# ming71/rotate-yolov3

Measured on AMD Instinct MI355X. Metric: images/sec fwd+bwd at 608^2 (train step, backend=hip), higher is better.
Workload: dtype bf16; 1 GPU; configs[3]: Darknet-53 train step (fwd + riou loss + bwd + grad all-reduce + SGD), bs=64/GPU 608x608, synthetic HRSC-shaped targets; global_batch=64, parallelism=dp1, gradients=250 MB fp32 in 4 flat buckets, fp32 on the wire

## Files before the change

rotate-yolov3_amd/csrc/conv.hip:

```cpp
#include <cstring>

#include <mutex>

#include "conv_common.h"

namespace ryolo_detail {
thread_local int *g_conv_choice = nullptr;
}

using namespace ryolo_detail;

namespace {

template <int KS, int BM, int BN, int WGM, int WGN, int NSTAGE, bool FAST, bool GEN, bool BNRED = false>
__global__ void __launch_bounds__(WGM *WGN * 64) conv_igemm_kernel(const ConvParams p, const BnRed br = BnRed()) {
    constexpr int NW = WGM * WGN, NT = NW * 64;
    constexpr int WPIX = BM / WGM, WCH = BN / WGN, PF = WPIX / 16, CF = WCH / 16;
    constexpr int A_BYTES = BM * BK * 2, B_BYTES = BN * BK * 2, STAGE = A_BYTES + B_BYTES;
    constexpr int A_PPW = (BM / 8) / NW, B_PPW = (BN / 8) / NW;
    static_assert(A_PPW >= 1 && B_PPW >= 1, "tile too small for the wave count");
    constexpr int SROW = BN * 2 + 16;
    static_assert(BM * SROW + WGM * 2 * BN * 4 <= NSTAGE * STAGE, "staging tile + statistics slots must fit in the operand buffers");
    constexpr int LOADS_PER_STAGE = A_PPW + B_PPW;

// ... 1992 lines not shown

int ryolo_conv_pack_job_fill(ryolo_pack_job *host_jobs , const float *w_oihw, int Cout, int Cin, int ksize,
                             int stride, int Cin_pad, void *packed_fwd, void *packed_dgrad ) {
    if (!host_jobs || !w_oihw || !packed_fwd || Cout <= 0 || Cin <= 0 || Cin_pad < Cin || (ksize != 1 && ksize != 3) ||
        (stride != 1 && stride != 2))
        return -1;
    int n = 0;
    {
        ryolo_pack_job &j = host_jobs[n++];
        j = ryolo_pack_job{};
        j.src = w_oihw; j.dst = packed_fwd; j.kind = 0; j.Cout = Cout; j.Cin = Cin; j.KS = ksize; j.Cin_pad = Cin_pad;
        j.Kpad = (ksize * ksize * Cin_pad + BK - 1) / BK * BK;
        j.rows = (Cout + 127) / 128 * 128;
        j.block_begin = 0; j.block_end = (j.rows + PK_ROWS - 1) / PK_ROWS;
        if (Cin * ksize * ksize > PK_LDS) return -1;
    }
    if (packed_dgrad) {
        if (ryolo_conv_packed_dgrad_bytes(Cout, Cin, ksize, stride) == 0) return -1;
        char *dst = (char *)packed_dgrad;
        for (int cls = 0; cls < (stride == 1 ? 1 : 4); cls++) {
            int dy[9], dx[9], khs[9], kws[9];
            const int nt = dgrad_classes(ksize, stride, (ksize - 1) / 2, cls, dy, dx, khs, kws);
            ryolo_pack_job &j = host_jobs[n++];
            j = ryolo_pack_job{};
            j.src = w_oihw; j.dst = dst; j.kind = 1; j.Cout = Cout; j.Cin = Cin; j.KS = ksize; j.ntaps = nt;
            for (int t = 0; t < nt; t++) { j.khs[t] = khs[t]; j.kws[t] = kws[t]; }
            j.Kpad = (nt * Cout + BK - 1) / BK * BK;
            j.rows = (Cin + 127) / 128 * 128;
            j.block_begin = 0; j.block_end = (j.rows / PK_CI) * ((Cout + PK_CO - 1) / PK_CO);
            dst += ((size_t)j.rows * j.Kpad + 128) * 2;
        }
        if (dgrad_xfusable(Cout, Cin, ksize, stride)) {
            for (int a = 0; a < 2; a++) {
                int dy[9], dx[9], khs[9], k0[9], k1[9];
                const int nt = dgrad_xfused_class(a, dy, dx, khs, k0, k1);
                ryolo_pack_job &j = host_jobs[n++];
                j = ryolo_pack_job{};
                j.src = w_oihw; j.dst = dst; j.kind = 2; j.Cout = Cout; j.Cin = Cin; j.KS = ksize; j.ntaps = nt;
                for (int t = 0; t < nt; t++) { j.khs[t] = khs[t]; j.kws[t] = (k0[t] + 1) | ((k1[t] + 1) << 4); }
                j.Kpad = (nt * Cout + BK - 1) / BK * BK;
                j.rows = (2 * Cin + 127) / 128 * 128;
                j.block_begin = 0; j.block_end = (j.rows / PK_CI) * ((Cout + PK_CO - 1) / PK_CO);
                dst += ((size_t)j.rows * j.Kpad + 128) * 2;
            }
        }
    }
    return n;
}

int ryolo_conv_pack_batch(const ryolo_pack_job *device_jobs, int njobs, int total_blocks, void *stream) {
    if (!device_jobs || njobs <= 0 || total_blocks <= 0) return RYOLO_EINVAL;
    hipLaunchKernelGGL(pack_batch_kernel, dim3((unsigned)total_blocks), dim3(256), 0, (hipStream_t)stream, device_jobs, njobs);
    return hipGetLastError() == hipSuccess ? RYOLO_OK : RYOLO_ELAUNCH;
}

int ryolo_conv_dgrad_tap_table(int ksize, int stride, int *host_out ) {
    if (!host_out || (ksize != 1 && ksize != 3) || (stride != 1 && stride != 2)) return RYOLO_EINVAL;
    for (int i = 0; i < 72; i++) host_out[i] = 0;
    for (int cls = 0; cls < (stride == 1 ? 1 : 4); cls++) {
        int dy[9], dx[9];
        dgrad_classes(ksize, stride, (ksize - 1) / 2, cls, dy, dx, host_out + cls * 18, host_out + cls * 18 + 9);
    }
    return RYOLO_OK;
}

int ryolo_conv_pack_weights_dgrad(const float *w_oihw, int Cout, int Cin, int ksize, int stride, void *packed,
                                  const int *taps_table , void *stream_) {
    if (!w_oihw || !packed || !taps_table || ryolo_conv_packed_dgrad_bytes(Cout, Cin, ksize, stride) == 0) return RYOLO_EINVAL;
    hipStream_t stream = (hipStream_t)stream_;
    const int rows = (Cin + 127) / 128 * 128;
    char *dst = (char *)packed;
    for (int cls = 0; cls < (stride == 1 ? 1 : 4); cls++) {
        int dy[9], dx[9], kk[18];
        const int nt = dgrad_classes(ksize, stride, (ksize - 1) / 2, cls, dy, dx, kk, kk + 9);
        const int Kpad = (nt * Cout + BK - 1) / BK * BK;
        const size_t total = (size_t)rows * Kpad + 128;
        const int nb = (int)((total + 255) / 256 < 4096 ? (total + 255) / 256 : 4096);
        hipLaunchKernelGGL(pack_dgrad_kernel, dim3(nb), dim3(256), 0, stream, w_oihw, Cout, Cin, ksize, nt,
                           taps_table + cls * 18, Kpad, rows, (__bf16 *)dst);
        dst += total * 2;
    }
    if (dgrad_xfusable(Cout, Cin, ksize, stride)) {
        const int rows2 = (2 * Cin + 127) / 128 * 128;
        for (int a = 0; a < 2; a++) {
            int dy[9], dx[9];
            XfTaps tp;
            const int nt = dgrad_xfused_class(a, dy, dx, tp.khs, tp.kw0, tp.kw1);
            for (int t = nt; t < 9; t++) { tp.khs[t] = 0; tp.kw0[t] = -1; tp.kw1[t] = -1; }
            const int Kpad = (nt * Cout + BK - 1) / BK * BK;
            const size_t total = (size_t)rows2 * Kpad + 128;
            const int nb = (int)((total + 255) / 256 < 4096 ? (total + 255) / 256 : 4096);
            hipLaunchKernelGGL(pack_dgrad_xfused_kernel, dim3(nb), dim3(256), 0, stream, w_oihw, Cout, Cin, nt, tp, Kpad, rows2,
                               (__bf16 *)dst);
            dst += total * 2;
        }
    }
    return hipGetLastError() == hipSuccess ? RYOLO_OK : RYOLO_ELAUNCH;
}

static int bnreduce_plan_tiles(const ryolo_conv_desc *d) {
    if (d->stride != 1 || (d->tile & 0xff) || d->in_cstride != d->Cin || (d->Cin & 7)) return 0;
    int knob = 1;
    {
        const char *e = tune(TUNE_BN_REDUCE_TILES);
        if (e) knob = atoi(e);
        if (knob == 0) return 0;
    }
    void *fake = (void *)(uintptr_t)4096;
    const BnRed *sv_b = g_bnred;
    const int sv_m = g_bnred_mode;
    int *sv_c = g_conv_choice;
    BnRed br{};
    int natural = -1, fused = -1;
    g_bnred = nullptr;
    g_conv_choice = &natural;
    int rc = ryolo_conv2d_dgrad(d, fake, d->Cout, fake, (const float *)fake, (const float *)fake, fake, 1, nullptr);
    if (rc == RYOLO_OK) {
        g_bnred = &br;
        g_bnred_mode = 3;
        g_conv_choice = &fused;
        rc = ryolo_conv2d_dgrad(d, fake, d->Cout, fake, (const float *)fake, (const float *)fake, fake, 1, nullptr);
    }
    g_bnred = sv_b;
    g_bnred_mode = sv_m;
    g_conv_choice = sv_c;
    if (rc != RYOLO_OK || natural != fused) return 0;
    const int tile = fused - RYOLO_CONV_KERNEL_IGEMM;
    const int bm = tile == 1 ? 128 : ((tile == 2 || tile == 3) ? 256 : 0);
    if (!bm) return 0;
    if (tile == 3) return 0;
    if (tile == 1 && knob == 2) return 0;
    const long long M = (long long)d->N * d->H * d->W;
    return (int)((M + bm - 1) / bm);
}

static int bnreduce_plan_mq128(const ryolo_conv_desc *d) {
    if (d->stride != 1 || (d->tile & 0xff) || d->in_cstride != d->Cin || (d->Cin & 127) || mq128_knob() <= 0) return 0;
    void *fake = (void *)(uintptr_t)4096;
    const BnRed *sv_b = g_bnred;
    int *sv_c = g_conv_choice;
    int natural = -1;
    g_bnred = nullptr;
    g_conv_choice = &natural;
    const int rc = ryolo_conv2d_dgrad(d, fake, d->Cout, fake, (const float *)fake, (const float *)fake, fake, 1, nullptr);
    g_bnred = sv_b;
    g_conv_choice = sv_c;
    if (rc != RYOLO_OK || (natural != RYOLO_CONV_KERNEL_MQ128 && natural != RYOLO_CONV_KERNEL_MQ64)) return 0;
    ConvParams q;
    q.M = (int)((long long)d->N * d->H * d->W);
    q.Cout = d->Cin;
    return conv_mq128_grid(q, natural == RYOLO_CONV_KERNEL_MQ128 ? 128 : 64);
}

static int bnreduce_plan(const ryolo_conv_desc *d, int *mode) {
    *mode = 0;
    if (validate(d) != RYOLO_OK) return 0;
    {
        const int r = bnreduce_plan_mq128(d);
        if (r > 0) {
            *mode = 4;
            return r;
        }
    }
    auto tiles = [&]() {
        const int r = bnreduce_plan_tiles(d);
        if (r > 0) *mode = 3;
        return r;
    };
    if (d->ksize != 1 || d->stride != 1 || d->pad != 0) return tiles();
    if ((d->Cin & 127) || (d->Cout & 63) || (d->tile & 0xff)) return tiles();
    const long long M = (long long)d->N * d->H * d->W;
    int g_pw = 0;
    {
        ConvParams q;
        q.Cin = d->Cout; q.Kpad = (d->Cout + BK - 1) / BK * BK; q.Cout = d->Cin; q.pw_grid_cap = 0;
        const int g = conv_pw_disabled() ? 0 : conv_pw_grid(q);
        if (g > 0 && d->in_cstride == d->Cin && ((unsigned long long)(M + 1024 * 128) * d->Cout) * 2ull < 0x7fffff00ull &&
            ((unsigned long long)M * d->Cin) * 2ull < 0x7fffff00ull)
            g_pw = g;
    }
    const long long mt = (M + 127) / 128, nt = d->Cin / 128, T = mt * nt;
    const int grid = (2 * cu_count()) & ~7;
    const long long dmax = d->W > d->H ? d->W : d->H;
    const bool persist_ok = !(grid < 8 || 2 * T < 5 * (long long)grid || mt * 128 * dmax >= 0x100000000ll || T * nt >= 0x100000000ll) &&
                            ((unsigned long long)M * d->Cout) * 2ull < 0x7fffff00ull;
    if (g_pw > 0 && (d->Cout == 128 || !persist_ok)) {
        *mode = 1;
        return g_pw;
    }
    if (persist_ok) {
        *mode = 2;
        return grid;
    }
    return tiles();
}

int ryolo_conv2d_dgrad_bnreduce_rows(const ryolo_conv_desc *d) {
    int mode;
    return bnreduce_plan(d, &mode);
}

int ryolo_conv2d_dgrad_bnreduce(const ryolo_conv_desc *d, const void *dz, int dz_cstride, const void *packed_dgrad, const float *ones,
                                const float *zeros, void *dx, int accumulate, const void *z, int z_cstride, const float *scale,
                                const float *shift, const float *mean, const float *invstd, const float *slope, float *part,
                                void *stream_) {
    int mode = 0;
    if (!bnreduce_plan(d, &mode) || !z || (z_cstride & 7) || z_cstride < d->Cin || !scale || !shift || !mean || !invstd ||
        !slope || !part || d->in_cstride != d->Cin)
        return RYOLO_EINVAL;
    BnRed br;
    br.z = (const __bf16 *)z; br.z_cs = z_cstride; br.scale = scale; br.shift = shift; br.mean = mean; br.invstd = invstd;
    br.slope = slope; br.part = part;
    g_bnred = &br;
    g_bnred_mode = mode;
    const int rc = ryolo_conv2d_dgrad(d, dz, dz_cstride, packed_dgrad, ones, zeros, dx, accumulate, stream_);
    g_bnred = nullptr;
    return rc;
}

int ryolo_conv2d_dgrad(const ryolo_conv_desc *d , const void *dz, int dz_cstride,
                       const void *packed_dgrad, const float *ones, const float *zeros, void *dx, int accumulate,
                       void *stream_) {
    if (validate(d) != RYOLO_OK || !dz || !packed_dgrad || !ones || !zeros || !dx) return RYOLO_EINVAL;
    if (d->stride != 1 && !(d->stride == 2 && d->ksize == 3 && d->pad == 1)) return RYOLO_EINVAL;
    if ((dz_cstride & 7) || dz_cstride < d->Cout) return RYOLO_EINVAL;
    const int Ho = (d->H + 2 * d->pad - d->ksize) / d->stride + 1, Wo = (d->W + 2 * d->pad - d->ksize) / d->stride + 1;
    const int rows = (d->Cin + 127) / 128 * 128;
    const char *wsrc = (const char *)packed_dgrad;
    const bool xfuse = dgrad_xfusable(d->Cout, d->Cin, d->ksize, d->stride) && d->pad == 1 && (d->W & 1) == 0 &&
                       d->in_cstride == d->Cin && !(d->tile & 0x8000);
    if (xfuse) wsrc += dgrad_classic_bytes(d->Cout, d->Cin, d->ksize, d->stride);
    if (!g_bnred && d->ksize == 3 && d->pad == 1 && ((d->Cin == 32 && d->Cout == 64) || (d->Cin == 64 && d->Cout == 128 && d->stride == 2)) &&
        !(d->tile & 0x80ff)) {
        const char *e = tune(TUNE_STEM_DGRAD);
        const int knob = e ? atoi(e) : 3;
        if (knob & (d->Cout == 64 ? 1 : 2)) {
            const int nt_out = (long long)d->N * d->H * d->W * d->Cin * 2 >= nt_out_min_bytes() ? 1 : 0;
            const unsigned long long dzb = (((unsigned long long)d->N * Ho * Wo - 1) * dz_cstride + d->Cout) * 2ull;
            const unsigned long long dxb = (((unsigned long long)d->N * d->H * d->W - 1) * d->in_cstride + d->Cin) * 2ull;
            if (dzb < 0x7fffff00ull && dxb < 0x7fffff00ull) {
                RYOLO_CONV_DRY_RUN(RYOLO_CONV_KERNEL_STEM_DGRAD);
                const int rc = launch_conv_stem_dgrad(d->Cout, d->stride, dz, dz_cstride, packed_dgrad, dx, d->in_cstride, accumulate, d->N, d->H,
                                                      d->W, nt_out, cu_count(), (hipStream_t)stream_);
                if (rc != RYOLO_EINVAL) return rc;
            }
        }
    }
    const int ncls = d->stride == 1 ? 1 : (xfuse ? 2 : 4);
    const int wrows = xfuse ? (2 * d->Cin + 127) / 128 * 128 : rows;
    for (int cls = 0; cls < ncls; cls++) {
        int dy[9], dxx[9], khs[9], kws[9];
        const int nt = xfuse ? dgrad_xfused_class(cls, dy, dxx, khs, kws, kws)
                             : dgrad_classes(d->ksize, d->stride, d->pad, cls, dy, dxx, khs, kws);
        ConvParams p;
        p.x = (const __bf16 *)dz;
        p.w = (const __bf16 *)wsrc;
        p.scale = ones; p.shift = zeros;
        p.res = accumulate ? (const __bf16 *)dx : nullptr;
        p.y = (__bf16 *)dx;
        p.N = d->N; p.H = Ho; p.W = Wo; p.Cin = d->Cout; p.in_cs = dz_cstride;
        p.Cout = d->Cin; p.out_cs = d->in_cstride; p.res_cs = d->in_cstride;
        p.K = nt * d->Cout;
        p.Kpad = (p.K + BK - 1) / BK * BK;
        p.act = RYOLO_ACT_LINEAR; p.slope = 0.f; p.ups = 1; p.nt = 0;
        p.cin_log2 = ilog2_exact(d->Cout);
        p.ntaps = nt;
        if (d->stride == 1) {
            p.stride = 1; p.pad = d->ksize - 1 - d->pad;
            p.Ho = d->H; p.Wo = d->W;
            for (int t = 0; t < nt; t++) { p.tap_dy[t] = dy[t]; p.tap_dx[t] = dxx[t]; }
            p.os = 1; p.osx = 1; p.ooy = 0; p.oox = 0; p.OH = d->H; p.OW = d->W;
        } else if (xfuse) {
            const int a = cls;
            p.stride = 1; p.pad = 0;
            p.Cout = 2 * d->Cin; p.out_cs = 2 * d->in_cstride; p.res_cs = 2 * d->in_cstride;
            p.Ho = (d->H - a + 1) / 2; p.Wo = d->W / 2;
            for (int t = 0; t < nt; t++) { p.tap_dy[t] = dy[t]; p.tap_dx[t] = dxx[t]; }
            p.os = 2; p.osx = 1; p.ooy = a; p.oox = 0; p.OH = d->H; p.OW = d->W / 2;
            if (p.Ho <= 0 || p.Wo <= 0) { wsrc += ((size_t)wrows * p.Kpad + 128) * 2; continue; }
        } else {
            const int a = cls >> 1, b = cls & 1;
            p.stride = 1; p.pad = 0;
            p.Ho = (d->H - a + 1) / 2; p.Wo = (d->W - b + 1) / 2;
            for (int t = 0; t < nt; t++) { p.tap_dy[t] = dy[t]; p.tap_dx[t] = dxx[t]; }
            p.os = 2; p.osx = 2; p.ooy = a; p.oox = b; p.OH = d->H; p.OW = d->W;
            if (p.Ho <= 0 || p.Wo <= 0) { wsrc += ((size_t)rows * p.Kpad + 128) * 2; continue; }
        }
        for (int t = nt; t < 9; t++) { p.tap_dy[t] = 0; p.tap_dx[t] = 0; }
        p.M = (int)((long long)d->N * p.Ho * p.Wo);
        const unsigned long long xb = (((unsigned long long)d->N * Ho * Wo - 1) * dz_cstride + d->Cout) * 2ull;
        const unsigned long long wb = ((unsigned long long)wrows * p.Kpad + 128) * 2ull;
        p.fast = (d->Cout % BK == 0) && xb < 0x7fffff00ull && wb < 0x7fffff00ull;
        p.taps2 = 0;
        if (!p.fast && (d->stride != 1 || (d->ksize == 3 && p.cin_log2 < 0))) return RYOLO_EINVAL;
        p.x_bytes = (unsigned)(p.fast ? xb : 0);
        p.w_bytes = (unsigned)(p.fast ? wb : 0);
        p.stat_part = nullptr; p.stat_cpad = 0;
        p.no_persist = (d->tile & 0x200) ? 1 : 0;
        p.force_persist = 0;
        p.pw_grid_cap = (d->tile & 0xff) == 13 ? (d->tile >> 16) & 0xff : 0;
        p.ntiles = 0; p.magic_wo = p.magic_ho = p.magic_nt = 0;
        p.nt_out = (long long)d->N * d->H * d->W * d->Cin * 2 >= nt_out_min_bytes() ? 1 : 0;
        const int pick = (d->tile & 0xff);
        const int rc = dispatch(p, d->ksize, pick, (hipStream_t)stream_);
        if (rc != RYOLO_OK) return rc;
        wsrc += ((size_t)wrows * p.Kpad + 128) * 2;
    }
    return RYOLO_OK;
}

}
```

rotate-yolov3_amd/csrc/conv_common.h:

```cpp
#pragma once
#include <hip/hip_runtime.h>
#include <stdint.h>
#include <stdlib.h>

#include "../../include/ryolo.h"

namespace ryolo_detail {

typedef __attribute__((ext_vector_type(8))) __bf16 bf16x8;
typedef __attribute__((ext_vector_type(4))) __bf16 bf16x4;
typedef __attribute__((ext_vector_type(2))) __bf16 bf16x2;
typedef __attribute__((ext_vector_type(4))) float f32x4;
typedef __attribute__((ext_vector_type(4))) unsigned int u32x4;
typedef __attribute__((address_space(3))) void *lds_vp;
typedef const __attribute__((address_space(1))) void *glb_vp;

constexpr int BK = 64;
constexpr long long NT_OUT_MIN_BYTES = 128ll << 20;
constexpr int STAT_ROWS = 128;

struct ConvParams {
    const __bf16 *x;
    const __bf16 *w;
    const float *scale;
    const float *shift;
    const __bf16 *res;
    __bf16 *y;
    int N, H, W, Cin, in_cs;
    int Ho, Wo, Cout, out_cs, res_cs;
    int stride, pad;
    int K, Kpad, M;
    int cin_log2;
    int act;
    float slope;
    int ups;
    int nt;
    unsigned x_bytes, w_bytes;
    int fast;
    int taps2;
    int no_persist;
    int force_persist;
    int ntaps;
    int tap_dy[9], tap_dx[9];
    int os, ooy, oox, OH, OW;
    int osx;
    int ntiles;
    unsigned magic_wo, magic_ho, magic_nt;
    int use_magic;
    unsigned y_bytes, res_bytes;
    double *stat_part;
    int stat_cpad;
    int nt_out;
    int reg3;
    int korder = 0;
    int dbg0, dbg1;
    int pw_nb, pw_mb;
    unsigned *trace;
    int pw_grid_cap;
};

struct BnRed {
    const __bf16 *z;
    int z_cs;
    const float *scale, *shift, *mean, *invstd;
    const float *slope;
    float *part;
    unsigned z_bytes = 0;
};

__device__ __forceinline__ float mish(float v) {
    const float e = __expf(fminf(v, 20.f));
    const float n = (1.f + e) * (1.f + e);
    return v * (n - 1.f) / (n + 1.f);
}

__device__ __forceinline__ float row16_sum(float v) {
#if defined(__HIP_DEVICE_COMPILE__)
    v += __builtin_bit_cast(float, __builtin_amdgcn_update_dpp(0, __builtin_bit_cast(int, v), 0xB1, 0xF, 0xF, true));
    v += __builtin_bit_cast(float, __builtin_amdgcn_update_dpp(0, __builtin_bit_cast(int, v), 0x4E, 0xF, 0xF, true));
    v += __builtin_bit_cast(float, __builtin_amdgcn_update_dpp(0, __builtin_bit_cast(int, v), 0x141, 0xF, 0xF, true));
    v += __builtin_bit_cast(float, __builtin_amdgcn_update_dpp(0, __builtin_bit_cast(int, v), 0x140, 0xF, 0xF, true));
#endif
    return v;
}

template <int O>
__device__ __forceinline__ float lane_xor_sum(float v) {
#if defined(__HIP_DEVICE_COMPILE__)
    if constexpr (O == 4) {
        v += __builtin_bit_cast(float, __builtin_amdgcn_update_dpp(0, __builtin_bit_cast(int, v), 0x124, 0xF, 0xF, true));
    } else if constexpr (O == 8) {
        v += __builtin_bit_cast(float, __builtin_amdgcn_update_dpp(0, __builtin_bit_cast(int, v), 0x128, 0xF, 0xF, true));
    } else if constexpr (O == 16) {
        const unsigned u = __builtin_bit_cast(unsigned, v);
        const auto s = __builtin_amdgcn_permlane16_swap(u, u, false, false);
        v = __builtin_bit_cast(float, (unsigned)s[0]) + __builtin_bit_cast(float, (unsigned)s[1]);
    } else {
        static_assert(O == 32, "partner distance");
        const unsigned u = __builtin_bit_cast(unsigned, v);
        const auto s = __builtin_amdgcn_permlane32_swap(u, u, false, false);
        v = __builtin_bit_cast(float, (unsigned)s[0]) + __builtin_bit_cast(float, (unsigned)s[1]);
    }
#endif
    return v;
}
template <int CPR>
__device__ __forceinline__ float lane_class_sum(float v) {
    if constexpr (CPR <= 4) v = lane_xor_sum<4>(v);
    if constexpr (CPR <= 8) v = lane_xor_sum<8>(v);
    v = lane_xor_sum<16>(v);
    return lane_xor_sum<32>(v);
}

__device__ __forceinline__ void buffer_load_lds16(const void *base, unsigned bytes, char *lds, int voffset, int soffset) {
#if defined(__HIP_DEVICE_COMPILE__)
    const __amdgpu_buffer_rsrc_t rsrc = __builtin_amdgcn_make_buffer_rsrc(const_cast<void *>(base), 0, bytes, 0x00020000);
    __builtin_amdgcn_raw_ptr_buffer_load_lds(rsrc, (lds_vp)lds, 16, voffset, soffset, 0, 0);
#endif
}

template <int AUX = 0>
__device__ __forceinline__ void buffer_store16_soff(u32x4 v, __amdgpu_buffer_rsrc_t rsrc, int voffset, int soffset) {
#if defined(__HIP_DEVICE_COMPILE__)
    __builtin_amdgcn_raw_buffer_store_b128(v, rsrc, voffset, soffset, AUX);
    asm volatile("s_nop 1" ::"v"(v));
#endif
}

__device__ __forceinline__ int udiv_magic(int n, unsigned magic) {
    return magic ? (int)__umulhi((unsigned)n, magic) : n;
}

__device__ __forceinline__ void split_pixel(int m, int Wo, int Ho, unsigned magic_wo, unsigned magic_ho, int use_magic, int &wo,
                                            int &ho, int &img) {
    if (use_magic) {
        const int t = udiv_magic(m, magic_wo);
        wo = m - t * Wo;
        img = udiv_magic(t, magic_ho);
        ho = t - img * Ho;
    } else {
        const int t = m / Wo;
        wo = m % Wo;
        ho = t % Ho;
        img = t / Ho;
    }
}


extern thread_local int *g_conv_choice;
#define RYOLO_CONV_DRY_RUN(code)          \
    do {                                  \
        if (ryolo_detail::g_conv_choice) { \
            *ryolo_detail::g_conv_choice = (code); \
            return RYOLO_OK;              \
        }                                 \
    } while (0)

int launch_conv_mp(ConvParams &p, int bm , int variant, hipStream_t stream);
int conv_mp_pick_bm(const ConvParams &p);
bool conv_mp_eligible(const ConvParams &p);
int launch_conv_mq(ConvParams &p, int variant, hipStream_t stream);
bool conv_mq128_eligible(const ConvParams &p);
int conv_mq128_grid(const ConvParams &p, int bm);
int launch_conv_mq128(ConvParams &p, int bm, const BnRed *bnred, hipStream_t stream);
bool conv_stem_eligible(const ConvParams &p, int ksize);
int launch_conv_stem(ConvParams &p, int cus, hipStream_t stream);
bool conv_stem64_eligible(const ConvParams &p, int ksize);
int launch_conv_stem64(ConvParams &p, int cus, hipStream_t stream);
int launch_conv0_halo(ConvParams &p, const float *slope_dev, int round_z, int cus, hipStream_t stream);
int launch_conv_stem_dgrad(int cdz, int stride, const void *dz, int dz_cs, const void *w_classes, void *dx, int dx_cs, int accumulate, int N,
                           int H, int W, int nt_out, int cus, hipStream_t stream);
int conv_stem_pair_kind(const ryolo_conv_desc *first, const ryolo_conv_desc *second, int shortcut_from_input);
int launch_conv_stem_pair(int kind, ConvParams &p , const void *x, unsigned x_bytes, int in_cs, int H, int W,
                          const void *w_first, int kpad_first, const float *scale_first, const float *shift_first, int act_first,
                          float slope_first, int cus, hipStream_t stream);
bool conv_pw_eligible(const ConvParams &p, int ksize);
bool conv_pw_preferred(const ConvParams &p);
int conv_pw_grid(const ConvParams &p);
int launch_conv_pw(ConvParams &p, const void *bnred , hipStream_t stream);
bool conv_pw_decode_supported(const ConvParams &p, int na, int no);
int launch_conv_pw_decode(ConvParams &p, float *io, long long io_img_rows, long long io_row0, float *pout, const float *anchors, int na, int no,
                          float stride, float cf, int arc, hipStream_t stream);
#ifdef RYOLO_MP_ABLATION
int ryolo_mp_ablation_variant(int slot);
#endif

enum TuneKey { TUNE_CONV3X3 = 0, TUNE_CONV1X1, TUNE_RNMS_TILES, TUNE_MQ_KORDER, TUNE_BN_REDUCE_TILES, TUNE_STEM_DGRAD, TUNE_COUNT };
const char *tune(TuneKey k);
#ifdef RYOLO_MP_ABLATION
inline const char *abl_env(const char *name) { return getenv(name); }
#else
inline const char *abl_env(const char *) { return nullptr; }
#endif

}
```

rotate-yolov3_amd/csrc/conv_stem.hip:

```cpp
#include <type_traits>

#include "conv_common.h"

namespace ryolo_detail {
namespace {

template <int N> using ic = std::integral_constant<int, N>;

constexpr int TW = 32;
constexpr int CIN = 32, COUT = 64, CG = COUT / 16;

template <int S>
struct Patch {
    static constexpr int TH = S == 1 ? 8 : 4;
    static constexpr int PH = (TH - 1) * S + 3, PW = (TW - 1) * S + 3, NPIX = PH * PW;
    static constexpr int NPIECE = (NPIX + 15) / 16;
    static constexpr int PPW = (NPIECE + 3) / 4;
    static constexpr int BUF = PPW * 4 * 1024;
    static constexpr int BYTES = 2 * BUF;
    static constexpr int GPW = TH * TW / 16 / 4;
};

__device__ __forceinline__ int chunk_swz(int pcol) { return (pcol ^ (pcol >> 2)) & 3; }

// ... 705 lines not shown
                }
            }
            f32x4 acc[2][2];
#pragma unroll
            for (int u = 0; u < 2; u++)
#pragma unroll
                for (int cg = 0; cg < 2; cg++) acc[u][cg] = f32x4{0.f, 0.f, 0.f, 0.f};
#pragma unroll
            for (int t = 0; t < 9; t++) {
                const int kh = t / 3, kw = t - 3 * kh;
#pragma unroll
                for (int ks = 0; ks < 2; ks++) {
                    bf16x8 xf[2];
#pragma unroll
                    for (int u = 0; u < 2; u++) {
                        const int pcol = u * 16 + fr + kw;
                        const int q = (jr + kh) * PW + pcol;
                        xf[u] = *(const bf16x8 *)(patch + q * 128 + (((ks * 4 + g) ^ swz(pcol)) << 4));
                    }
#pragma unroll
                    for (int u = 0; u < 2; u++)
#pragma unroll
                        for (int cg = 0; cg < 2; cg++)
                            acc[u][cg] = __builtin_amdgcn_mfma_f32_16x16x32_bf16(wfr[t][ks][cg], xf[u], acc[u][cg], 0, 0, 0);
                }
            }
#pragma unroll
            for (int u = 0; u < 2; u++) {
                unsigned o2[2][2];
#pragma unroll
                for (int cg = 0; cg < 2; cg++) {
                    bf16x4 o;
                    if constexpr (STATS) {
#pragma unroll
                        for (int rr = 0; rr < 4; rr++) {
                            o[rr] = (__bf16)acc[u][cg][rr];
                            const float qv = ok_[u] ? (float)o[rr] : 0.f;
                            st_sum[cg][rr] += qv;
                            st_sq[cg][rr] += qv * qv;
                        }
                    } else {
#pragma unroll
                        for (int rr = 0; rr < 4; rr++) {
                            float v = acc[u][cg][rr] * sc[cg][rr] + sh[cg][rr];
                            if constexpr (ACT == RYOLO_ACT_LEAKY) v = v > 0.f ? v : v * slope;
                            else if constexpr (ACT == RYOLO_ACT_MISH) v = mish(v);
                            o[rr] = (__bf16)v;
                        }
                    }
                    const uint2 uu = __builtin_bit_cast(uint2, o);
                    o2[cg][0] = uu.x;
                    o2[cg][1] = uu.y;
                }
#if defined(__HIP_DEVICE_COMPILE__)
#pragma unroll
                for (int d = 0; d < 2; d++) {
                    auto sw = __builtin_amdgcn_permlane16_swap(o2[0][d], o2[1][d], false, false);
                    o2[0][d] = sw[0];
                    o2[1][d] = sw[1];
                }
#endif
                u32x4 outv = u32x4{o2[0][0], o2[0][1], o2[1][0], o2[1][1]};
                if constexpr (!STATS) {
                    if (p.res) {
                        bf16x8 ov = __builtin_bit_cast(bf16x8, outv);
#pragma unroll
                        for (int e = 0; e < 8; e++) ov[e] = (__bf16)((float)ov[e] + (float)rv[u][e]);
                        outv = __builtin_bit_cast(u32x4, ov);
                    }
                }
                if (ok_[u]) {
                    u32x4 *dst = (u32x4 *)(p.y + (mbase + u * 16) * p.out_cs + co0 + run0);
                    if (p.nt_out) __builtin_nontemporal_store(outv, dst);
                    else *dst = outv;
                }
            }
        }
    }
    if constexpr (STATS) {
        float ta = 0.f, tb = 0.f;
#pragma unroll
        for (int cg = 0; cg < 2; cg++)
#pragma unroll
            for (int rr = 0; rr < 4; rr++) {
                const float a = row16_sum(st_sum[cg][rr]), b = row16_sum(st_sq[cg][rr]);
                if (fr == cg * 4 + rr) {
                    ta = a;
                    tb = b;
                }
            }
        if (fr < 8) {
            const int ch = co0 + (fr >> 2) * 16 + g * 4 + (fr & 3);
            double *row = p.stat_part + (size_t)(blockIdx.x % STAT_ROWS) * 2 * p.stat_cpad;
            atomicAdd(row + ch, (double)ta);
            atomicAdd(row + p.stat_cpad + ch, (double)tb);
        }
    }
}

template <bool STATS, int ACT>
int launch_stem64(ConvParams &p, int grid, int tiles_x, int tiles_y, int ntiles, hipStream_t stream) {
    hipLaunchKernelGGL((conv3x3_c64_halo_kernel<STATS, ACT>), dim3((unsigned)grid), dim3(256), c64::BYTES, stream, p, tiles_x, tiles_y, ntiles);
    return hipGetLastError() == hipSuccess ? RYOLO_OK : RYOLO_ELAUNCH;
}

template <int S, bool STATS>
int launch_stem(ConvParams &p, int grid, int tiles_x, int tiles_y, int ntiles, hipStream_t stream) {
    constexpr int smem = Patch<S>::BYTES;
    static bool attr_done = false;
    if (!attr_done) {
        if (smem > 64 * 1024 && hipFuncSetAttribute((const void *)conv3x3_c32_halo_kernel<S, STATS>,
                                                    hipFuncAttributeMaxDynamicSharedMemorySize, smem) != hipSuccess)
            return RYOLO_ELAUNCH;
        attr_done = true;
    }
    hipLaunchKernelGGL((conv3x3_c32_halo_kernel<S, STATS>), dim3((unsigned)grid), dim3(256), smem, stream, p, tiles_x, tiles_y, ntiles);
    return hipGetLastError() == hipSuccess ? RYOLO_OK : RYOLO_ELAUNCH;
}

}

bool conv_stem_eligible(const ConvParams &p, int ksize) {
    return ksize == 3 && p.Cin == CIN && p.Cout == COUT && p.pad == 1 && (p.stride == 1 || p.stride == 2) && p.fast && p.os == 1 &&
           p.ups == 1 && p.ntaps == 9 && (p.in_cs & 7) == 0 && (p.out_cs & 7) == 0 && (!p.res || (p.res_cs & 7) == 0) &&
           !(p.stat_part && p.res) && (long long)p.N * p.H * p.W * p.in_cs * 2 < 0x7fffff00ll;
}

bool conv_stem64_eligible(const ConvParams &p, int ksize) {
    return ksize == 3 && p.Cin == c64::CIN && p.Cout == c64::COUT && p.pad == 1 && p.stride == 1 && p.fast && p.os == 1 &&
           p.ups == 1 && p.ntaps == 9 && (p.in_cs & 7) == 0 && (p.out_cs & 7) == 0 && (!p.res || (p.res_cs & 7) == 0) &&
           !(p.stat_part && p.res) && (long long)p.N * p.H * p.W * p.in_cs * 2 < 0x7fffff00ll;
}

int launch_conv_stem64(ConvParams &p, int cus, hipStream_t stream) {
    const int tiles_x = (p.Wo + c64::TWX - 1) / c64::TWX, tiles_y = (p.Ho + c64::TH - 1) / c64::TH;
    const long long nt = (long long)p.N * tiles_x * tiles_y;
    if (nt > 0x7fffffffll) return RYOLO_EINVAL;
    RYOLO_CONV_DRY_RUN(RYOLO_CONV_KERNEL_STEM64);
    int grid = (2 * cus) & ~7;
    if (grid < 8) grid = 8;
    if (p.stat_part) return launch_stem64<true, RYOLO_ACT_LINEAR>(p, grid, tiles_x, tiles_y, (int)nt, stream);
    if (p.act == RYOLO_ACT_LEAKY) return launch_stem64<false, RYOLO_ACT_LEAKY>(p, grid, tiles_x, tiles_y, (int)nt, stream);
    if (p.act == RYOLO_ACT_MISH) return launch_stem64<false, RYOLO_ACT_MISH>(p, grid, tiles_x, tiles_y, (int)nt, stream);
    return launch_stem64<false, RYOLO_ACT_LINEAR>(p, grid, tiles_x, tiles_y, (int)nt, stream);
}

struct DgTile128 {
    static constexpr int TH = 8, TW = 32;
    static constexpr int PH = TH / 2 + 1, PW = TW / 2 + 1, NPIX = PH * PW;
    static constexpr int NPIECE = (NPIX + 3) / 4;
    static constexpr int PPW = (NPIECE + 3) / 4, BUF = PPW * 4 * 1024;
};

__global__ void __launch_bounds__(256, 2) dgrad3x3_s2_c128_kernel(const DgS2Params p) {
    using T = DgTile128;
    extern __shared__ __attribute__((aligned(16))) char smem[];
    const int tid = threadIdx.x, lane = tid & 63;
    const int wave = __builtin_amdgcn_readfirstlane(tid >> 6);
    const int fr = lane & 15, g = lane >> 4;
    const int q8 = p.ntiles >> 3, r8 = p.ntiles & 7, xcd = blockIdx.x & 7, loc = blockIdx.x >> 3, nloc = gridDim.x >> 3;
    const int start = xcd < r8 ? xcd * (q8 + 1) : r8 * (q8 + 1) + (xcd - r8) * q8;
    const int len = q8 + (xcd < r8 ? 1 : 0);
    bf16x8 wf[9][4];
    {
        constexpr int NCLS = 4;
        const __bf16 *img = p.w;
        int t0 = 0;
#pragma unroll
        for (int cls = 0; cls < NCLS; cls++) {
            const int nt = cls == 0 ? 1 : (cls == 3 ? 4 : 2), kpad = nt * 128;
#pragma unroll
            for (int t = 0; t < 4; t++) {
                if (t >= nt) break;
#pragma unroll
                for (int ks = 0; ks < 4; ks++) wf[t0 + t][ks] = *(const bf16x8 *)(img + (size_t)(wave * 16 + fr) * kpad + t * 128 + ks * 32 + g * 8);
            }
            t0 += nt;
            img += 128 * kpad + 128;
        }
    }
    const int tiles_img = p.tiles_x * p.tiles_y;
    auto fill = [&](int id, char *buf) {
        const int img = id / tiles_img, rem = id - img * tiles_img;
        const int ty = rem / p.tiles_x, tx = rem - ty * p.tiles_x;
        const int h0 = ty * (T::TH / 2), w0 = tx * (T::TW / 2);
#pragma unroll 2
        for (int j = 0; j < T::PPW; j++) {
            const int piece = wave * T::PPW + j;
            const int q = piece * 4 + (lane >> 4);
            const int prow = q / T::PW, pcol = q - prow * T::PW;
            const int ho = h0 + prow, wo = w0 + pcol;
            const bool ok = q < T::NPIX && (unsigned)ho < (unsigned)p.Ho && (unsigned)wo < (unsigned)p.Wo;
            const int chunk = (lane & 15) ^ (pcol & 15);
            const int off = (((img * p.Ho + ho) * p.Wo + wo) * p.dz_cs + chunk * 8) * 2;
            buffer_load_lds16(p.dz, p.dz_bytes, buf + piece * 1024, ok ? off : (int)0x80000000, 0);
        }
    };
    typedef __attribute__((ext_vector_type(2))) unsigned int u32x2;
    int cur = 0;
    if (loc < len) fill(start + loc, smem);
    for (int i = loc; i < len; i += nloc) {
        const int id = start + i;
        const int img = id / tiles_img, rem = id - img * tiles_img;
        const int ty = rem / p.tiles_x, tx = rem - ty * p.tiles_x;
        const int hi0 = ty * T::TH, wi0 = tx * T::TW;
        asm volatile("s_waitcnt vmcnt(0)" ::: "memory");
        __syncthreads();
        if (i + nloc < len) fill(id + nloc, smem + (cur ^ 1) * T::BUF);
        const char *patch = smem + cur * T::BUF;
        cur ^= 1;
        auto group = [&](auto Ac, auto Bc, auto T0c, int r) {
            constexpr int A = decltype(Ac)::value, B = decltype(Bc)::value, T0 = decltype(T0c)::value;
            constexpr int NTA = A ? 2 : 1, NTB = B ? 2 : 1;
            const int hi = hi0 + r, wi = wi0 + 2 * fr + B;
            const bool ok = hi < p.H && wi < p.W;
            const size_t m = ((size_t)img * p.H + hi) * p.W + wi;
            const int coff = wave * 16 + g * 4;
            u32x2 rv = u32x2{0u, 0u};
            if (p.res && ok) rv = *(const u32x2 *)(p.res + m * p.dx_cs + coff);
            f32x4 acc = f32x4{0.f, 0.f, 0.f, 0.f};
#pragma unroll
            for (int ta = 0; ta < NTA; ta++)
#pragma unroll
                for (int tb = 0; tb < NTB; tb++) {
                    const int prow = (r - A) / 2 + (A ? ta : 0), pcol = fr + (B ? tb : 0);
                    const char *px = patch + (prow * T::PW + pcol) * 256;
                    const int sw = pcol & 15;
#pragma unroll
                    for (int ks = 0; ks < 4; ks++) {
                        const bf16x8 xf = *(const bf16x8 *)(px + (((g + 4 * ks) ^ sw) << 4));
                        acc = __builtin_amdgcn_mfma_f32_16x16x32_bf16(wf[T0 + ta * NTB + tb][ks], xf, acc, 0, 0, 0);
                    }
                }
            bf16x4 o;
#pragma unroll
            for (int rr = 0; rr < 4; rr++) o[rr] = (__bf16)acc[rr];
            if (p.res) {
                const bf16x4 rb = __builtin_bit_cast(bf16x4, rv);
#pragma unroll
                for (int rr = 0; rr < 4; rr++) o[rr] = (__bf16)((float)o[rr] + (float)rb[rr]);
            }
            if (ok) {
                u32x2 *dst = (u32x2 *)(p.dx + m * p.dx_cs + coff);
                if (p.nt_out) __builtin_nontemporal_store(__builtin_bit_cast(u32x2, o), dst);
                else *dst = __builtin_bit_cast(u32x2, o);
            }
        };
        {
#pragma unroll
            for (int rp = 0; rp < T::TH / 2; rp++) {
                group(ic<0>{}, ic<0>{}, ic<0>{}, 2 * rp);
                group(ic<0>{}, ic<1>{}, ic<1>{}, 2 * rp);
                group(ic<1>{}, ic<0>{}, ic<3>{}, 2 * rp + 1);
                group(ic<1>{}, ic<1>{}, ic<5>{}, 2 * rp + 1);
            }
        }
    }
}

int launch_conv_stem_dgrad(int cdz, int stride, const void *dz, int dz_cs, const void *w_classes, void *dx, int dx_cs, int accumulate, int N,
                           int H, int W, int nt_out, int cus, hipStream_t stream) {
    const int Ho = stride == 2 ? (H - 1) / 2 + 1 : H, Wo = stride == 2 ? (W - 1) / 2 + 1 : W;
    const unsigned long long dzb = (((unsigned long long)N * Ho * Wo - 1) * dz_cs + cdz) * 2ull;
    if ((stride != 1 && stride != 2) || (cdz != 64 && !(cdz == 128 && stride == 2)) || dzb >= 0x7fffff00ull || (dz_cs & 7) || (dx_cs & 7) || dz_cs < cdz ||
        dx_cs < cdz / 2)
        return RYOLO_EINVAL;
    DgS2Params q;
    q.dz = (const __bf16 *)dz; q.dz_bytes = (unsigned)dzb; q.dz_cs = dz_cs; q.w = (const __bf16 *)w_classes;
    q.dx = (__bf16 *)dx; q.dx_cs = dx_cs; q.res = accumulate ? (const __bf16 *)dx : nullptr;
    q.H = H; q.W = W; q.Ho = Ho; q.Wo = Wo;
    const int th = cdz == 64 ? (stride == 2 ? DgTile<2>::TH : DgTile<1>::TH) : DgTile128::TH;
    const int tw = cdz == 64 ? (stride == 2 ? DgTile<2>::TW : DgTile<1>::TW) : DgTile128::TW;
    q.tiles_x = (W + tw - 1) / tw; q.tiles_y = (H + th - 1) / th;
    const long long nt = (long long)q.tiles_x * q.tiles_y * N;
    if (nt >= 0x7fffffff) return RYOLO_EINVAL;
    q.ntiles = (int)nt; q.nt_out = nt_out;
    int grid = (2 * cus) & ~7;
    if (grid < 8) grid = 8;
    if (cdz == 64) {
        if (stride == 2) hipLaunchKernelGGL(dgrad3x3_c64_kernel<2>, dim3((unsigned)grid), dim3(256), 2 * DgTile<2>::BUF, stream, q);
        else hipLaunchKernelGGL(dgrad3x3_c64_kernel<1>, dim3((unsigned)grid), dim3(256), 2 * DgTile<1>::BUF, stream, q);
    } else {
        hipLaunchKernelGGL(dgrad3x3_s2_c128_kernel, dim3((unsigned)grid), dim3(256), 2 * DgTile128::BUF, stream, q);
    }
    return hipGetLastError() == hipSuccess ? RYOLO_OK : RYOLO_ELAUNCH;
}

int launch_conv0_halo(ConvParams &p, const float *slope_dev, int round_z, int cus, hipStream_t stream) {
    if (!p.y || p.stat_part) return RYOLO_EINVAL;
    const int tiles_x = (p.Wo + C0_TW - 1) / C0_TW, tiles_y = (p.Ho + C0_TH - 1) / C0_TH;
    const long long nt = (long long)p.N * tiles_x * tiles_y;
    if (nt > 0x7fffffffll) return RYOLO_EINVAL;
    int grid = (4 * cus) & ~7;
    if (grid < 8) grid = 8;
    return launch_conv0_halo_t(p, slope_dev, round_z, p.act, grid, tiles_x, tiles_y, (int)nt, stream);
}

int launch_conv_stem(ConvParams &p, int cus, hipStream_t stream) {
    const int th = p.stride == 1 ? Patch<1>::TH : Patch<2>::TH;
    const int tiles_x = (p.Wo + TW - 1) / TW, tiles_y = (p.Ho + th - 1) / th;
    const long long nt = (long long)p.N * tiles_x * tiles_y;
    if (nt > 0x7fffffffll) return RYOLO_EINVAL;
    RYOLO_CONV_DRY_RUN(RYOLO_CONV_KERNEL_STEM);
    int grid = (2 * cus) & ~7;
    if (grid < 8) grid = 8;
    if (p.stat_part) return p.stride == 1 ? launch_stem<1, true>(p, grid, tiles_x, tiles_y, (int)nt, stream)
                                          : launch_stem<2, true>(p, grid, tiles_x, tiles_y, (int)nt, stream);
    return p.stride == 1 ? launch_stem<1, false>(p, grid, tiles_x, tiles_y, (int)nt, stream)
                         : launch_stem<2, false>(p, grid, tiles_x, tiles_y, (int)nt, stream);
}

static int launch_pair(ConvParams &p, const PairFirst &f, int cus, hipStream_t stream) {
    using G = PairGeom;
    const int tiles_x = (p.Wo + TW - 1) / TW, tiles_y = (p.Ho + G::P::TH - 1) / G::P::TH;
    const long long nt = (long long)p.N * tiles_x * tiles_y;
    if (nt > 0x7fffffffll) return RYOLO_EINVAL;
    static bool attr_done = false;
    if (!attr_done) {
        if (G::BYTES > 64 * 1024 && hipFuncSetAttribute((const void *)conv_stem_pair_kernel, hipFuncAttributeMaxDynamicSharedMemorySize,
                                                        G::BYTES) != hipSuccess)
            return RYOLO_ELAUNCH;
        attr_done = true;
    }
    int grid = (2 * cus) & ~7;
    if (grid < 8) grid = 8;
    hipLaunchKernelGGL(conv_stem_pair_kernel, dim3((unsigned)grid), dim3(256), G::BYTES, stream, p, f, tiles_x, tiles_y, (int)nt);
    return hipGetLastError() == hipSuccess ? RYOLO_OK : RYOLO_ELAUNCH;
}

int conv_stem_pair_kind(const ryolo_conv_desc *a, const ryolo_conv_desc *b, int shortcut_from_input) {
    if (!a || !b || a->upsample != 1 || b->upsample != 1 || a->N != b->N) return 0;
    const int aho = (a->H + 2 * a->pad - a->ksize) / a->stride + 1, awo = (a->W + 2 * a->pad - a->ksize) / a->stride + 1;
    if (aho != b->H || awo != b->W || a->Cout != b->Cin || b->Cin != CIN || b->Cout != COUT || b->ksize != 3 || b->pad != 1) return 0;
    if ((long long)a->N * a->H * a->W * a->in_cstride * 2 >= 0x7fffff00ll) return 0;
    if (a->ksize == 1 && a->stride == 1 && a->pad == 0 && a->Cin == 64 && b->stride == 1 && shortcut_from_input && (a->in_cstride & 7) == 0) return 2;
    return 0;
}

int launch_conv_stem_pair(int kind, ConvParams &p, const void *x, unsigned x_bytes, int in_cs, int H, int W, const void *w_first, int kpad_first,
                          const float *scale_first, const float *shift_first, int act_first, float slope_first, int cus, hipStream_t stream) {
    PairFirst f;
    f.x = (const __bf16 *)x; f.w = (const __bf16 *)w_first; f.scale = scale_first; f.shift = shift_first; f.x_bytes = x_bytes;
    f.in_cs = in_cs; f.Kpad = kpad_first; f.act = act_first; f.slope = slope_first; f.H = H; f.W = W;
    (void)kind;
    return launch_pair(p, f, cus, stream);
}

}
```

Before: 1381 images/s.

## Fuse BN/leaky-ReLU backward reduction into stride-2 stem dgrad kernel

Adds a BN-reduce mode to the specialized 3x3 stride-2 C128 stem dgrad kernel. The kernel now loads the pre-activation z, applies the leaky-ReLU gradient mask, and accumulates the per-channel BN backward partial sums in-kernel, writing per-block partials. Previously that layer either used the generic dgrad path with reduction or ran a separate reduction pass. The change avoids re-reading dx and z, at the cost of extra register pressure and z loads inside the stem kernel.

```diff
diff --git a/rotate-yolov3_amd/csrc/conv.hip b/rotate-yolov3_amd/csrc/conv.hip
--- a/rotate-yolov3_amd/csrc/conv.hip
+++ b/rotate-yolov3_amd/csrc/conv.hip
@@ -2168,9 +2168,32 @@
     return conv_mq128_grid(q, natural == RYOLO_CONV_KERNEL_MQ128 ? 128 : 64);
 }
 
+static int bnreduce_plan_stem(const ryolo_conv_desc *d) {
+    if (d->ksize != 3 || d->pad != 1 || d->stride != 2 || d->Cin != 64 || d->Cout != 128 || (d->tile & 0x80ff) || d->in_cstride != d->Cin) return 0;
+    {
+        const char *e = tune(TUNE_BN_REDUCE_TILES);
+        if (e && atoi(e) == 0) return 0;
+        const char *s = tune(TUNE_STEM_DGRAD);
+        if (!((s ? atoi(s) : 3) & 2)) return 0;
+    }
+    const int Ho = (d->H - 1) / 2 + 1, Wo = (d->W - 1) / 2 + 1;
+    const unsigned long long dzb = (((unsigned long long)d->N * Ho * Wo - 1) * d->Cout + d->Cout) * 2ull;
+    const unsigned long long dxb = (((unsigned long long)d->N * d->H * d->W - 1) * d->in_cstride + d->Cin) * 2ull;
+    if (dzb >= 0x7fffff00ull || dxb >= 0x7fffff00ull) return 0;
+    if ((long long)((d->W + 31) / 32) * ((d->H + 7) / 8) * d->N >= 0x7fffffff) return 0;
+    return conv_stem_dgrad_grid(cu_count());
+}
+
 static int bnreduce_plan(const ryolo_conv_desc *d, int *mode) {
     *mode = 0;
     if (validate(d) != RYOLO_OK) return 0;
+    {
+        const int r = bnreduce_plan_stem(d);
+        if (r > 0) {
+            *mode = 5;
+            return r;
+        }
+    }
     {
         const int r = bnreduce_plan_mq128(d);
         if (r > 0) {
@@ -2246,8 +2269,9 @@
     const bool xfuse = dgrad_xfusable(d->Cout, d->Cin, d->ksize, d->stride) && d->pad == 1 && (d->W & 1) == 0 &&
                        d->in_cstride == d->Cin && !(d->tile & 0x8000);
     if (xfuse) wsrc += dgrad_classic_bytes(d->Cout, d->Cin, d->ksize, d->stride);
-    if (!g_bnred && d->ksize == 3 && d->pad == 1 && ((d->Cin == 32 && d->Cout == 64) || (d->Cin == 64 && d->Cout == 128 && d->stride == 2)) &&
-        !(d->tile & 0x80ff)) {
+    const bool stem_red = g_bnred && g_bnred_mode == 5;
+    if ((!g_bnred || stem_red) && d->ksize == 3 && d->pad == 1 &&
+        ((d->Cin == 32 && d->Cout == 64 && !stem_red) || (d->Cin == 64 && d->Cout == 128 && d->stride == 2)) && !(d->tile & 0x80ff)) {
         const char *e = tune(TUNE_STEM_DGRAD);
         const int knob = e ? atoi(e) : 3;
         if (knob & (d->Cout == 64 ? 1 : 2)) {
@@ -2257,11 +2281,12 @@
             if (dzb < 0x7fffff00ull && dxb < 0x7fffff00ull) {
                 RYOLO_CONV_DRY_RUN(RYOLO_CONV_KERNEL_STEM_DGRAD);
                 const int rc = launch_conv_stem_dgrad(d->Cout, d->stride, dz, dz_cstride, packed_dgrad, dx, d->in_cstride, accumulate, d->N, d->H,
-                                                      d->W, nt_out, cu_count(), (hipStream_t)stream_);
-                if (rc != RYOLO_EINVAL) return rc;
-            }
-        }
-    }
+                                                      d->W, nt_out, cu_count(), stem_red ? g_bnred : nullptr, (hipStream_t)stream_);
+                if (rc != RYOLO_EINVAL || stem_red) return rc;
+            }
+        }
+    }
+    if (stem_red) return RYOLO_EINVAL;
     const int ncls = d->stride == 1 ? 1 : (xfuse ? 2 : 4);
     const int wrows = xfuse ? (2 * d->Cin + 127) / 128 * 128 : rows;
     for (int cls = 0; cls < ncls; cls++) {
diff --git a/rotate-yolov3_amd/csrc/conv_common.h b/rotate-yolov3_amd/csrc/conv_common.h
--- a/rotate-yolov3_amd/csrc/conv_common.h
+++ b/rotate-yolov3_amd/csrc/conv_common.h
@@ -169,7 +169,8 @@
 int launch_conv_stem64(ConvParams &p, int cus, hipStream_t stream);
 int launch_conv0_halo(ConvParams &p, const float *slope_dev, int round_z, int cus, hipStream_t stream);
 int launch_conv_stem_dgrad(int cdz, int stride, const void *dz, int dz_cs, const void *w_classes, void *dx, int dx_cs, int accumulate, int N,
-                           int H, int W, int nt_out, int cus, hipStream_t stream);
+                           int H, int W, int nt_out, int cus, const BnRed *bnred, hipStream_t stream);
+int conv_stem_dgrad_grid(int cus);
 int conv_stem_pair_kind(const ryolo_conv_desc *first, const ryolo_conv_desc *second, int shortcut_from_input);
 int launch_conv_stem_pair(int kind, ConvParams &p , const void *x, unsigned x_bytes, int in_cs, int H, int W,
                           const void *w_first, int kpad_first, const float *scale_first, const float *shift_first, int act_first,
diff --git a/rotate-yolov3_amd/csrc/conv_stem.hip b/rotate-yolov3_amd/csrc/conv_stem.hip
--- a/rotate-yolov3_amd/csrc/conv_stem.hip
+++ b/rotate-yolov3_amd/csrc/conv_stem.hip
@@ -881,7 +881,8 @@
     static constexpr int PPW = (NPIECE + 3) / 4, BUF = PPW * 4 * 1024;
 };
 
-__global__ void __launch_bounds__(256, 2) dgrad3x3_s2_c128_kernel(const DgS2Params p) {
+template <bool BNRED>
+__global__ void __launch_bounds__(256, 2) dgrad3x3_s2_c128_kernel(const DgS2Params p, const BnRed br) {
     using T = DgTile128;
     extern __shared__ __attribute__((aligned(16))) char smem[];
     const int tid = threadIdx.x, lane = tid & 63;
@@ -926,8 +927,31 @@
         }
     };
     typedef __attribute__((ext_vector_type(2))) unsigned int u32x2;
+    float bs1[4], bs2[4], bs3[4];
+    const float bn_slope = BNRED ? br.slope[0] : 0.f;
+    const float *bn_cst = (const float *)(smem + 2 * T::BUF);
+#pragma unroll
+    for (int rr = 0; rr < 4; rr++) bs1[rr] = bs2[rr] = bs3[rr] = 0.f;
+    if constexpr (BNRED) {
+        if (tid < 192) ((float *)(smem + 2 * T::BUF))[tid] = (tid < 64 ? br.scale : (tid < 128 ? br.shift : br.mean))[tid & 63];
+    }
+    u32x2 zq[4] = {u32x2{0u, 0u}, u32x2{0u, 0u}, u32x2{0u, 0u}, u32x2{0u, 0u}};
+    auto zreq = [&](int id2, int r, int B) -> u32x2 {
+        const int img2 = id2 / tiles_img, rem2 = id2 - img2 * tiles_img;
+        const int ty2 = rem2 / p.tiles_x, tx2 = rem2 - ty2 * p.tiles_x;
+        const int hi = ty2 * T::TH + r, wi = tx2 * T::TW + 2 * fr + B;
+        u32x2 v = u32x2{0u, 0u};
+        if (hi < p.H && wi < p.W) v = *(const u32x2 *)(br.z + (((size_t)img2 * p.H + hi) * p.W + wi) * br.z_cs + wave * 16 + g * 4);
+        return v;
+    };
     int cur = 0;
-    if (loc < len) fill(start + loc, smem);
+    if (loc < len) {
+        if constexpr (BNRED) {
+#pragma unroll
+            for (int k = 0; k < 4; k++) zq[k] = zreq(start + loc, k >> 1, k & 1);
+        }
+        fill(start + loc, smem);
+    }
     for (int i = loc; i < len; i += nloc) {
         const int id = start + i;
         const int img = id / tiles_img, rem = id - img * tiles_img;
@@ -938,9 +962,9 @@
         if (i + nloc < len) fill(id + nloc, smem + (cur ^ 1) * T::BUF);
         const char *patch = smem + cur * T::BUF;
         cur ^= 1;
-        auto group = [&](auto Ac, auto Bc, auto T0c, int r) {
-            constexpr int A = decltype(Ac)::value, B = decltype(Bc)::value, T0 = decltype(T0c)::value;
-            constexpr int NTA = A ? 2 : 1, NTB = B ? 2 : 1;
+        auto group = [&](auto Ac, auto Bc, auto T0c, auto RPc) {
+            constexpr int A = decltype(Ac)::value, B = decltype(Bc)::value, T0 = decltype(T0c)::value, RP = decltype(RPc)::value;
+            constexpr int NTA = A ? 2 : 1, NTB = B ? 2 : 1, r = 2 * RP + A;
             const int hi = hi0 + r, wi = wi0 + 2 * fr + B;
             const bool ok = hi < p.H && wi < p.W;
             const size_t m = ((size_t)img * p.H + hi) * p.W + wi;
@@ -974,21 +998,63 @@
                 if (p.nt_out) __builtin_nontemporal_store(__builtin_bit_cast(u32x2, o), dst);
                 else *dst = __builtin_bit_cast(u32x2, o);
             }
+            if constexpr (BNRED) {
+                const f32x4 bsc = *(const f32x4 *)(bn_cst + coff), bsh = *(const f32x4 *)(bn_cst + 64 + coff), bmu = *(const f32x4 *)(bn_cst + 128 + coff);
+                if (ok) {
+                    const bf16x4 zb = __builtin_bit_cast(bf16x4, zq[2 * A + B]);
+#pragma unroll
+                    for (int rr = 0; rr < 4; rr++) {
+                        const float zf = (float)zb[rr], dv = (float)o[rr];
+                        const float u = zf * bsc[rr] + bsh[rr];
+                        float gq = dv;
+                        if (u <= 0.f) { gq = dv * bn_slope; bs3[rr] += dv * u; }
+                        bs2[rr] += gq * (zf - bmu[rr]);
+                        bs1[rr] += gq;
+                    }
+                }
+                if constexpr (RP + 1 < T::TH / 2) zq[2 * A + B] = zreq(id, r + 2, B);
+                else if (i + nloc < len) zq[2 * A + B] = zreq(id + nloc, A, B);
+                __builtin_amdgcn_sched_barrier(0);
+            }
         };
-        {
-#pragma unroll
-            for (int rp = 0; rp < T::TH / 2; rp++) {
-                group(ic<0>{}, ic<0>{}, ic<0>{}, 2 * rp);
-                group(ic<0>{}, ic<1>{}, ic<1>{}, 2 * rp);
-                group(ic<1>{}, ic<0>{}, ic<3>{}, 2 * rp + 1);
-                group(ic<1>{}, ic<1>{}, ic<5>{}, 2 * rp + 1);
-            }
-        }
-    }
+        auto rows2 = [&](auto rp) {
+            group(ic<0>{}, ic<0>{}, ic<0>{}, rp);
+            group(ic<0>{}, ic<1>{}, ic<1>{}, rp);
+            group(ic<1>{}, ic<0>{}, ic<3>{}, rp);
+            group(ic<1>{}, ic<1>{}, ic<5>{}, rp);
+        };
+        static_assert(T::TH / 2 == 4, "four row pairs per tile");
+        rows2(ic<0>{}); rows2(ic<1>{}); rows2(ic<2>{}); rows2(ic<3>{});
+    }
+    if constexpr (BNRED) {
+        const int coff = wave * 16 + g * 4;
+#pragma unroll
+        for (int rr = 0; rr < 4; rr++) bs2[rr] *= br.invstd[coff + rr];
+#pragma unroll
+        for (int k = 1; k < 16; k <<= 1)
+#pragma unroll
+            for (int rr = 0; rr < 4; rr++) {
+                bs1[rr] += __shfl_xor(bs1[rr], k, 64);
+                bs2[rr] += __shfl_xor(bs2[rr], k, 64);
+                bs3[rr] += __shfl_xor(bs3[rr], k, 64);
+            }
+        if (fr == 0) {
+            float *row = br.part + (size_t)blockIdx.x * 3 * 64 + coff;
+            *(f32x4 *)row = f32x4{bs1[0], bs1[1], bs1[2], bs1[3]};
+            *(f32x4 *)(row + 64) = f32x4{bs2[0], bs2[1], bs2[2], bs2[3]};
+            *(f32x4 *)(row + 128) = f32x4{bs3[0], bs3[1], bs3[2], bs3[3]};
+        }
+    }
+}
+
+int conv_stem_dgrad_grid(int cus) {
+    const int grid = (2 * cus) & ~7;
+    return grid < 8 ? 8 : grid;
 }
 
 int launch_conv_stem_dgrad(int cdz, int stride, const void *dz, int dz_cs, const void *w_classes, void *dx, int dx_cs, int accumulate, int N,
-                           int H, int W, int nt_out, int cus, hipStream_t stream) {
+                           int H, int W, int nt_out, int cus, const BnRed *bnred, hipStream_t stream) {
+    if (bnred && !(cdz == 128 && stride == 2)) return RYOLO_EINVAL;
     const int Ho = stride == 2 ? (H - 1) / 2 + 1 : H, Wo = stride == 2 ? (W - 1) / 2 + 1 : W;
     const unsigned long long dzb = (((unsigned long long)N * Ho * Wo - 1) * dz_cs + cdz) * 2ull;
     if ((stride != 1 && stride != 2) || (cdz != 64 && !(cdz == 128 && stride == 2)) || dzb >= 0x7fffff00ull || (dz_cs & 7) || (dx_cs & 7) || dz_cs < cdz ||
@@ -1004,13 +1070,14 @@
     const long long nt = (long long)q.tiles_x * q.tiles_y * N;
     if (nt >= 0x7fffffff) return RYOLO_EINVAL;
     q.ntiles = (int)nt; q.nt_out = nt_out;
-    int grid = (2 * cus) & ~7;
-    if (grid < 8) grid = 8;
+    const int grid = conv_stem_dgrad_grid(cus);
     if (cdz == 64) {
         if (stride == 2) hipLaunchKernelGGL(dgrad3x3_c64_kernel<2>, dim3((unsigned)grid), dim3(256), 2 * DgTile<2>::BUF, stream, q);
         else hipLaunchKernelGGL(dgrad3x3_c64_kernel<1>, dim3((unsigned)grid), dim3(256), 2 * DgTile<1>::BUF, stream, q);
     } else {
-        hipLaunchKernelGGL(dgrad3x3_s2_c128_kernel, dim3((unsigned)grid), dim3(256), 2 * DgTile128::BUF, stream, q);
+        if (bnred && ((((uintptr_t)bnred->part) & 15) || (bnred->z_cs & 3))) return RYOLO_EINVAL;
+        if (bnred) hipLaunchKernelGGL(dgrad3x3_s2_c128_kernel<true>, dim3((unsigned)grid), dim3(256), 2 * DgTile128::BUF + 3 * 64 * 4, stream, q, *bnred);
+        else hipLaunchKernelGGL(dgrad3x3_s2_c128_kernel<false>, dim3((unsigned)grid), dim3(256), 2 * DgTile128::BUF, stream, q, BnRed());
     }
     return hipGetLastError() == hipSuccess ? RYOLO_OK : RYOLO_ELAUNCH;
 }
```

Result: no change. 1370 images/s (-0.8%).
